# clawrim/gcn10

Measured on AMD Instinct MI355X. Metric: CN Gpixels/sec, higher is better.
Workload: dtype u8

## Files before the change

### gcn10_amd/csrc/gcn10_deflate_fused.hip

```cpp
#include <hip/hip_runtime.h>

#include <cstdint>
#include <cstring>

#include "gcn10_deflate_internal.hpp"
#include "gcn10_gpu.h"
#include "gcn10_gpu_internal.hpp"

using gcn10::as_stream;
using gcn10::fail;
using gcn10::u32x4;
using gcn10::use_device;
using namespace gcn10_deflate;

namespace {

constexpr int kGroup = 6;

struct FusedJob {
    const uint8_t *esa;
    const uint8_t *hx;
    const int32_t *cj;
    const uint8_t *class_of;
    uint16_t *tok;
// ... 1297 lines not shown
            const uint32_t at = (uint32_t)kMaxStream - 4u;
            o[at] = (uint8_t)(adler >> 24);
            o[at + 1] = (uint8_t)(adler >> 16);
            o[at + 2] = (uint8_t)(adler >> 8);
            o[at + 3] = (uint8_t)adler;
        }
        const uint8_t *val = class_val + job.sel[j] * 256;
        const uint32_t xc = (uint32_t)(t & 63) * 4u;
        for (int i = 0; i < kTile / 4; i++) {
            const int r = i * 4 + (t >> 6);
            const uint32_t c4 = class_pixels4(job, tx * kTile + xc, ty * kTile + (uint32_t)r, sh.class_of);
            uint8_t *dst = o + 2 + (r >> 7) * (5 + 32768) + 5 + (r & 127) * kTile + xc;
            dst[0] = val[c4 & 0xffu];
            dst[1] = val[(c4 >> 8) & 0xffu];
            dst[2] = val[(c4 >> 16) & 0xffu];
            dst[3] = val[c4 >> 24];
        }
    }
}

}

extern "C" {

int gcn10_gpu_deflate_fused_available(gcn10_gpu_ctx *ctx)
{
    return ctx && ctx->n_tables > 0 && ctx->n_classes > 0 ? 1 : 0;
}

int gcn10_gpu_deflate_fused_strip(gcn10_gpu_ctx *ctx, const uint8_t *esa, int W, int rows, const int32_t *cj,
                                  unsigned cond_mask, unsigned table_mask, uint8_t *arena_dev, size_t arena_cap,
                                  uint32_t *table_dev, unsigned long long *cursor_dev, gcn10_stream_t stream)
{
    int rc = use_device(ctx);
    if (rc)
        return rc;
    if (ctx->n_tables == 0)
        return fail(GCN10_E_STATE, "gcn10_gpu_deflate_fused_strip: call gcn10_gpu_set_tables first");
    if (ctx->n_classes == 0)
        return fail(GCN10_E_STATE, "gcn10_gpu_deflate_fused_strip: the lookup tables define more than 256 pixel "
                                   "classes; use gcn10_gpu_cn_strip + gcn10_gpu_deflate_strip");
    if (!ctx->d_hx || ctx->hx_W == 0 || (uint32_t)W != ctx->hx_W)
        return fail(GCN10_E_STATE, "gcn10_gpu_deflate_fused_strip: call gcn10_gpu_prepare_tile for W=%d first", W);
    if (W <= 0 || rows < 0 || cond_mask == 0 || (cond_mask & ~3u) || table_mask == 0 ||
        (table_mask >> ctx->n_tables))
        return fail(GCN10_E_INVAL, "gcn10_gpu_deflate_fused_strip: bad shape or masks");
    if (rows == 0)
        return GCN10_OK;
    if (!esa || !cj || !arena_dev || !table_dev || !cursor_dev)
        return fail(GCN10_E_INVAL, "gcn10_gpu_deflate_fused_strip: null pointer");
    if ((reinterpret_cast<uintptr_t>(arena_dev) & 15u) != 0)
        return fail(GCN10_E_INVAL, "gcn10_gpu_deflate_fused_strip: arena must be 16-byte aligned");

    FusedJob job;
    memset(&job, 0, sizeof job);
    job.esa = esa;
    job.hx = ctx->d_hx;
    job.cj = cj;
    job.class_of = ctx->d_class_of;
    job.hx_stride = ctx->hx_stride;
    job.hx_rows = ctx->hx_rows;
    job.seg_align = (uint32_t)ctx->arena_segment_align;
    for (int r = 0; r < GCN10_N_RASTERS; r++)
        if ((cond_mask >> (r / 9)) & 1u && (table_mask >> (r % 9)) & 1u)
            job.sel[job.n_sel++] = (uint8_t)r;
    job.t.arena = arena_dev;
    job.t.table = table_dev;
    job.t.cursor = cursor_dev;
    job.t.W = (uint32_t)W;
    job.t.rows = (uint32_t)rows;
    job.t.across = ((uint32_t)W + kTile - 1) / kTile;
    job.t.down = ((uint32_t)rows + kTile - 1) / kTile;
    if (arena_cap >= 0xfffffffeull)
        return fail(GCN10_E_INVAL, "tile encoder: an arena of %zu bytes does not fit 32-bit stream offsets "
                                   "(use fewer rows per strip)", arena_cap);
    job.t.arena_cap = arena_cap;
    const uint32_t positions = job.t.across * job.t.down;
    if ((uint64_t)positions * (uint64_t)(kMaxStream + kSlotAlign) >= 0xffffffffull)
        return fail(GCN10_E_INVAL, "tile encoder: %u tile positions in one strip (use fewer rows per strip)", positions);
    const uint64_t nblocks = (uint64_t)positions * job.n_sel;
    job.t.n_tiles = (uint32_t)nblocks;

    const size_t stats_bytes = ((size_t)nblocks * ((size_t)kHistWords * 4 + (size_t)kBookBytes) + 255) & ~(size_t)255;
    const size_t tok_bytes = (size_t)positions * kTokStride * sizeof(uint16_t);
    const size_t ntok_bytes = ((size_t)positions * sizeof(uint32_t) + 15) & ~(size_t)15;
    const size_t need = stats_bytes + tok_bytes + ntok_bytes + (size_t)nblocks * 8 + (size_t)job.n_sel * ((positions + 63u) / 64u) * 4;
    rc = gcn10::grow_workspace(&ctx->deflate_ws, &ctx->deflate_ws_cap, need);
    if (rc)
        return rc;
    job.t.hist = reinterpret_cast<uint32_t *>(ctx->deflate_ws);
    job.t.books = reinterpret_cast<uint8_t *>(ctx->deflate_ws) + (size_t)nblocks * kHistWords * 4;
    job.tok = reinterpret_cast<uint16_t *>(reinterpret_cast<uint8_t *>(ctx->deflate_ws) + stats_bytes);
    job.n_tok = reinterpret_cast<uint32_t *>(reinterpret_cast<uint8_t *>(ctx->deflate_ws) + stats_bytes + tok_bytes);
    job.t.sizes = table_dev;
    if (ctx->fused_emit != 0) {
        job.t.sizes = reinterpret_cast<uint32_t *>(reinterpret_cast<uint8_t *>(ctx->deflate_ws) + stats_bytes + tok_bytes + ntok_bytes);
        job.t.chunk_tot = job.t.sizes + (size_t)nblocks * 2;
        job.t.n_chunks = (positions + 63u) / 64u;
    }

    static_assert(sizeof(SharedFA) <= 80 * 1024, "two fused statistics workgroups per CU");
    static_assert(sizeof(SharedFA2) <= 80 * 1024, "two segment-parallel statistics workgroups (32 waves) per CU");
    static_assert(sizeof(SharedFC) <= 20 * 1024, "eight fused emit workgroups per CU");
    static_assert(sizeof(SharedFC2) <= 16 * 1024, "ten wave-independent emit workgroups per CU by LDS");
    if (!ctx->fused_ready) {
        HIP_TRY(hipFuncSetAttribute(reinterpret_cast<const void *>(fused_stats_kernel),
// ... 28 lines not shown
```

### gcn10_amd/csrc/gcn10_gpu.hip

```cpp

#include <hip/hip_runtime.h>
#include <unistd.h>
#include <hip/hip_ext.h>

#include <cstdarg>
#include <cstdint>
#include <cstdio>
#include <cstdlib>
#include <cstring>
#include <new>

#include "gcn10_gpu.h"
#include "gcn10_gpu_internal.hpp"

using gcn10::as_stream;
using gcn10::fail;
using gcn10::u32x4;
using gcn10::use_device;

namespace {

constexpr int kThreads = 256;
constexpr int kPxPerLane = 16;
constexpr int kChunk = kThreads * kPxPerLane;
// ... 358 lines not shown
            }
        }
    }
}

__global__ __launch_bounds__(kThreads) void stream_copy_kernel(const u32x4 *in, u32x4 *out, uint32_t nvec,
                                                               uint32_t ntrips)
{
    uint32_t step, end;
    for (uint32_t trip = first_chunk(ntrips, step, end, true); trip < end; trip += step) {
        u32x4 v[2];
        uint32_t idx[2];
#pragma unroll
        for (int u = 0; u < 2; u++) {
            idx[u] = (trip * 2u + u) * (uint32_t)kThreads + threadIdx.x;
            v[u] = __builtin_nontemporal_load(in + (idx[u] < nvec ? idx[u] : 0u));
        }
#pragma unroll
        for (int u = 0; u < 2; u++)
            if (idx[u] < nvec)
                __builtin_nontemporal_store(v[u], out + idx[u]);
    }
}

__global__ __launch_bounds__(kThreads) void cn_strip_bytes(const StripParams p,
                                                           uint32_t cond_mask)
{
    __shared__ __attribute__((aligned(16))) uint8_t lut[kLut16Bytes];
    for (int i = threadIdx.x; i < kLut16Bytes; i += kThreads)
        lut[i] = p.lut[i];
    __syncthreads();

    const uint32_t stride = gridDim.x * blockDim.x;
    for (uint32_t i = blockIdx.x * blockDim.x + threadIdx.x; i < p.npix; i += stride) {
        const uint32_t y = i / p.W;
        const uint32_t x = i - y * p.W;
        const uint32_t lc = p.esa[i];
        const uint32_t cd = p.hx[(size_t)soil_row(p, y) * p.hx_stride + x];
        for (int c = 0; c < 2; c++) {
            if (!(cond_mask & (1u << c)))
                continue;
            const uint32_t s = (cd >> (4 * c)) & 0xfu;
            const uint8_t *row = lut + s * (uint32_t)kPlane16 + lc * 16u;
            for (int k = 0; k < 9; k++)
                if (p.table_mask & (1u << k))
                    p.out[c * 9 + k][i] = row[k];
        }
    }
}

constexpr uint32_t kExpandRows = 4;

template <bool VEC>
__global__ __launch_bounds__(kThreads) void expand_x_codes(const uint8_t *coarse,
                                                           uint32_t hsx, uint32_t hsy,
                                                           const int32_t *ci, uint32_t W,
                                                           uint8_t *hx, uint32_t hx_stride,
                                                           uint32_t *hx4, uint32_t *complex, uint32_t gen)
{
    const uint32_t x = (blockIdx.x * blockDim.x + threadIdx.x) * 16u;
    const uint32_t r0 = blockIdx.y * kExpandRows;
    if (x >= hx_stride || r0 >= hsy)
        return;
    const uint8_t pad = (uint8_t)(kInvalidPlane | (kInvalidPlane << 4));
    uint32_t cx[16];
    if (VEC && x + 16u <= W) {
        const u32x4 *civ = reinterpret_cast<const u32x4 *>(ci + x);
#pragma unroll
        for (int j = 0; j < 4; j++) {
            const u32x4 c4 = civ[j];
#pragma unroll
            for (int q = 0; q < 4; q++)
                cx[4 * j + q] = c4[q] < hsx ? c4[q] : hsx - 1u;
        }
    }
    else {
#pragma unroll
        for (int q = 0; q < 16; q++) {
            const uint32_t xx = x + q;
            const uint32_t c = xx < W ? (uint32_t)ci[xx] : 0u;
            cx[q] = xx < W ? (c < hsx ? c : hsx - 1u) : 0xffffffffu;
        }
    }
    const uint32_t c_lo = cx[0], c_hi = cx[15];
    const uint32_t r1 = r0 + kExpandRows < hsy ? r0 + kExpandRows : hsy;
    uint32_t split = 0;
    bool compact = true, in_set = true;
#pragma unroll
    for (int q = 0; q < 16; q++) {
        const bool lo = cx[q] == c_lo;
        in_set = in_set && (lo || cx[q] == c_hi);
        compact = compact && (lo ? split == (uint32_t)q : cx[q] == c_hi);
        split += lo && split == (uint32_t)q ? 1u : 0u;
    }
    const bool two = c_lo != 0xffffffffu && c_hi != 0xffffffffu && in_set;
    if (hx4 && x < W && !compact && *reinterpret_cast<volatile uint32_t *>(complex) != gen)
        *reinterpret_cast<volatile uint32_t *>(complex) = gen;
    for (uint32_t r = r0; r < r1; r++) {
        const uint8_t *row = coarse + (size_t)r * hsx;
        u32x4 o;
        if (two) {
            const uint32_t code_lo = soil_code(row[c_lo]), code_hi = soil_code(row[c_hi]);
#pragma unroll
            for (int j = 0; j < 4; j++) {
                uint32_t w = 0;
#pragma unroll
                for (int q = 0; q < 4; q++)
                    w |= (cx[4 * j + q] == c_lo ? code_lo : code_hi) << (8 * q);
                o[j] = w;
            }
        }
        else {
#pragma unroll
            for (int j = 0; j < 4; j++) {
                uint32_t w = 0;
#pragma unroll
                for (int q = 0; q < 4; q++) {
                    const uint32_t c = cx[4 * j + q];
                    const uint8_t code = c == 0xffffffffu ? pad : soil_code(row[c]);
                    w |= (uint32_t)code << (8 * q);
                }
                o[j] = w;
            }
        }
        __builtin_nontemporal_store(o, reinterpret_cast<u32x4 *>(hx + (size_t)r * hx_stride + x));
        if (hx4)
            __builtin_nontemporal_store(compact ? (o[0] & 0xffu) | ((o[3] >> 24) << 8) | (split << 16) : 0x00ff0000u,
                                        hx4 + (size_t)r * (hx_stride / 16u) + x / 16u);
    }
}

__global__ __launch_bounds__(kThreads) void resample_rows(const uint8_t *coarse,
                                                          uint32_t hsx,
                                                          const int32_t *ci,
                                                          const int32_t *cj, uint32_t W,
                                                          uint32_t rows, uint8_t *out)
{
    const size_t npix = (size_t)W * rows;
    const size_t stride = (size_t)gridDim.x * blockDim.x;
    for (size_t i = (size_t)blockIdx.x * blockDim.x + threadIdx.x; i < npix; i += stride) {
        const uint32_t y = (uint32_t)(i / W);
        const uint32_t x = (uint32_t)(i - (size_t)y * W);
        out[i] = coarse[(size_t)(uint32_t)cj[y] * hsx + (uint32_t)ci[x]];
    }
}

__device__ __forceinline__ uint8_t remap_soil(uint8_t h, bool drained)
{
    if (h >= 11 && h <= 14)
        return drained ? (uint8_t)4 : (uint8_t)(h - 10);
    return h;
}

__global__ __launch_bounds__(kThreads) void modify_hysogs_kernel(uint8_t *h, size_t npix,
                                                                 int drained,
                                                                 size_t head, size_t nvec)
{
    const size_t stride = (size_t)gridDim.x * blockDim.x;
    const size_t tid = (size_t)blockIdx.x * blockDim.x + threadIdx.x;
    u32x4 *body = reinterpret_cast<u32x4 *>(h + head);
    for (size_t v = tid; v < nvec; v += stride) {
        u32x4 in = body[v];
        u32x4 o;
#pragma unroll
        for (int j = 0; j < 4; j++) {
            uint32_t w = 0;
#pragma unroll
            for (int q = 0; q < 4; q++)
                w |= (uint32_t)remap_soil((uint8_t)(in[j] >> (8 * q)), drained != 0) << (8 * q);
            o[j] = w;
        }
        body[v] = o;
    }
    const size_t tail0 = head + nvec * 16;
    const size_t nscalar = head + (npix - tail0);
    for (size_t s = tid; s < nscalar; s += stride) {
        const size_t i = s < head ? s : tail0 + (s - head);
        h[i] = remap_soil(h[i], drained != 0);
    }
}

template <bool VEC>
// ... 106 lines not shown
    case 4:
        if (KIND == kLut1)
            return nt ? pick_by_mask<kLut1, 4, true>(cond_mask, all, pf) : pick_by_mask<kLut1, 4, false>(cond_mask, all, pf);
        return nullptr;
    default: return nullptr;
    }
}

strip_kernel_t pick_strip_kernel(bool single, unsigned cond_mask, bool all, int ilp, bool nt, bool pf)
{
    return single ? pick_by_ilp<kLut1>(cond_mask, all, ilp, nt, pf)
                  : pick_by_ilp<kLut16>(cond_mask, all, ilp, nt, pf);
}

}

namespace gcn10 {

thread_local char g_err[512] = "";

int fail(int code, const char *fmt, ...)
{
    va_list ap;
    va_start(ap, fmt);
    vsnprintf(g_err, sizeof g_err, fmt, ap);
    va_end(ap);
    return code;
}

int use_device(gcn10_gpu_ctx *ctx)
{
    if (!ctx)
        return fail(GCN10_E_INVAL, "null context");
    HIP_TRY(hipSetDevice(ctx->device));
    return GCN10_OK;
}

hipStream_t as_stream(gcn10_gpu_ctx *ctx, gcn10_stream_t s)
{
    return s ? reinterpret_cast<hipStream_t>(s) : ctx->main_stream;
}

int grow_workspace(void **ws, size_t *cap, size_t need)
{
    if (need <= *cap)
        return GCN10_OK;
    HIP_TRY(hipDeviceSynchronize());
    if (*ws)
        HIP_TRY(hipFree(*ws));
    *ws = nullptr;
    *cap = 0;
    HIP_TRY(hipMalloc(ws, need));
    *cap = need;
    return GCN10_OK;
}

}

namespace {

uint32_t stream_grid(const gcn10_gpu_ctx *ctx, uint64_t nchunks, int blocks_per_cu = 0)
{
    uint64_t cap = (uint64_t)ctx->n_cus * (blocks_per_cu > 0 ? blocks_per_cu : ctx->grid_blocks_per_cu);
    cap -= cap % 8u;
    if (cap < 8)
        cap = 8;
    uint64_t g = nchunks < cap ? nchunks : cap;
    return (uint32_t)(g ? g : 1);
}

}

extern "C" {

int gcn10_gpu_abi_version(void)
{
    return GCN10_GPU_ABI_VERSION;
}

const char *gcn10_gpu_last_error(void)
{
    return gcn10::g_err;
}

int gcn10_gpu_device_count(void)
{
    int n = 0;
    if (hipGetDeviceCount(&n) != hipSuccess)
        return 0;
    return n;
}

int gcn10_gpu_init(int device, gcn10_gpu_ctx **out)
{
    if (!out)
        return fail(GCN10_E_INVAL, "gcn10_gpu_init: null out pointer");
    *out = nullptr;
    int n = 0;
    hipError_t e = hipGetDeviceCount(&n);
    if (e != hipSuccess || n <= 0)
        return fail(GCN10_E_NODEVICE, "no HIP device visible (%s); this engine has no CPU fallback",
                    e != hipSuccess ? hipGetErrorString(e) : "device count 0");
    if (device < 0 || device >= n)
        return fail(GCN10_E_INVAL, "device %d out of range (0..%d)", device, n - 1);
    HIP_TRY(hipSetDevice(device));
    hipDeviceProp_t prop;
    HIP_TRY(hipGetDeviceProperties(&prop, device));
    if (strncmp(prop.gcnArchName, "gfx950", 6) != 0)
        return fail(GCN10_E_NODEVICE, "device %d is %s; this library carries gfx950 code only",
                    device, prop.gcnArchName);

    gcn10_gpu_ctx *ctx = new (std::nothrow) gcn10_gpu_ctx();
    if (!ctx)
        return fail(GCN10_E_NOMEM, "context allocation failed");
    ctx->device = device;
    ctx->n_cus = prop.multiProcessorCount;
    hipError_t e2 = hipStreamCreateWithFlags(&ctx->main_stream, hipStreamNonBlocking);
    if (e2 == hipSuccess)
        e2 = hipMalloc(reinterpret_cast<void **>(&ctx->d_lut16), kLut16Bytes);
    if (e2 == hipSuccess)
        e2 = hipMalloc(reinterpret_cast<void **>(&ctx->d_lut1), GCN10_N_TABLES * kLut1Bytes);
    if (e2 != hipSuccess) {
        int rc = fail(GCN10_E_HIP, "context setup: %s", hipGetErrorString(e2));
        gcn10_gpu_destroy(ctx);
        return rc;
    }
    *out = ctx;
    return GCN10_OK;
}

void gcn10_gpu_destroy(gcn10_gpu_ctx *ctx)
{
    if (!ctx)
        return;
    (void)hipSetDevice(ctx->device);
    if (ctx->main_stream) {
        (void)hipStreamSynchronize(ctx->main_stream);
        (void)hipStreamDestroy(ctx->main_stream);
    }
    if (ctx->d_lut16)
        (void)hipFree(ctx->d_lut16);
    if (ctx->d_lut1)
        (void)hipFree(ctx->d_lut1);
    if (ctx->d_hx_alloc)
        (void)hipFree(ctx->d_hx_alloc);
    if (ctx->deflate_ws)
        (void)hipFree(ctx->deflate_ws);
    if (ctx->inflate_ws)
        (void)hipFree(ctx->inflate_ws);
    if (ctx->lzw_ws)
        (void)hipFree(ctx->lzw_ws);
    if (ctx->d_class_of)
        (void)hipFree(ctx->d_class_of);
    delete ctx;
}

int gcn10_gpu_device_info(gcn10_gpu_ctx *ctx, char *name, size_t cap, size_t *hbm_bytes)
{
    int rc = use_device(ctx);
    if (rc)
        return rc;
    hipDeviceProp_t prop;
    HIP_TRY(hipGetDeviceProperties(&prop, ctx->device));
    if (name && cap)
        snprintf(name, cap, "%s (%s)", prop.name[0] ? prop.name : "AMD GPU", prop.gcnArchName);
    if (hbm_bytes)
        *hbm_bytes = prop.totalGlobalMem;
    return prop.multiProcessorCount;
}

int gcn10_gpu_pci_bus_id(int device, char *buf, size_t cap)
{
    if (!buf || cap < 13)
        return fail(GCN10_E_INVAL, "gcn10_gpu_pci_bus_id: buffer too small");
    HIP_TRY(hipDeviceGetPCIBusId(buf, (int)cap, device));
    return GCN10_OK;
}


int gcn10_gpu_malloc(gcn10_gpu_ctx *ctx, size_t bytes, void **dptr)
{
    int rc = use_device(ctx);
    if (rc)
        return rc;
    if (!dptr)
        return fail(GCN10_E_INVAL, "gcn10_gpu_malloc: null out pointer");
    *dptr = nullptr;
    HIP_TRY(hipMalloc(dptr, bytes ? bytes : 1));
    return GCN10_OK;
}

int gcn10_gpu_free(gcn10_gpu_ctx *ctx, void *dptr)
{
    int rc = use_device(ctx);
    if (rc)
        return rc;
    if (dptr)
        HIP_TRY(hipFree(dptr));
// ... 301 lines not shown
    return GCN10_OK;
}

int gcn10_gpu_calculate_cn(gcn10_gpu_ctx *ctx, const uint8_t *esa, const uint8_t *hsg,
                           size_t npix, int table_index, uint8_t *out, gcn10_stream_t stream)
{
    int rc = use_device(ctx);
    if (rc)
        return rc;
    if (ctx->n_tables == 0)
        return fail(GCN10_E_STATE, "gcn10_gpu_calculate_cn: call gcn10_gpu_set_tables first");
    if (table_index < 0 || table_index >= ctx->n_tables)
        return fail(GCN10_E_INVAL, "gcn10_gpu_calculate_cn: table %d not loaded (have %d)",
                    table_index, ctx->n_tables);
    if (npix == 0)
        return GCN10_OK;
    if (!esa || !hsg || !out)
        return fail(GCN10_E_INVAL, "gcn10_gpu_calculate_cn: null pointer");
    const uint8_t *img = ctx->d_lut1 + (size_t)table_index * kLut1Bytes;
    const bool vec = aligned16(esa) && aligned16(hsg) && aligned16(out);
    const uint64_t work = vec ? (npix / 16 + 2 * kThreads - 1) / (2 * kThreads) + 1
                              : (npix + kThreads - 1) / kThreads;
    const uint32_t grid = stream_grid(ctx, work);
    if (vec)
        hipLaunchKernelGGL(calculate_cn_kernel<true>, dim3(grid), dim3(kThreads), 0,
                           as_stream(ctx, stream), esa, hsg, npix, img, out);
    else
        hipLaunchKernelGGL(calculate_cn_kernel<false>, dim3(grid), dim3(kThreads), 0,
                           as_stream(ctx, stream), esa, hsg, npix, img, out);
    HIP_TRY(hipGetLastError());
    return GCN10_OK;
}


int gcn10_gpu_prepare_tile(gcn10_gpu_ctx *ctx, const uint8_t *coarse, int hsx, int hsy,
                           const int32_t *ci, int W, gcn10_stream_t stream)
{
    int rc = use_device(ctx);
    if (rc)
        return rc;
    if (hsx <= 0 || hsy <= 0 || W <= 0)
        return fail(GCN10_E_INVAL, "gcn10_gpu_prepare_tile: bad shape W=%d soil=%dx%d", W, hsx, hsy);
    if (!coarse || !ci)
        return fail(GCN10_E_INVAL, "gcn10_gpu_prepare_tile: null pointer");
    const uint32_t stride = (((uint32_t)W + 15u) & ~15u) + 16u;
    const size_t need = (size_t)stride * (size_t)hsy;
    if (need > ctx->hx_capacity) {
        HIP_TRY(hipDeviceSynchronize());
        if (ctx->d_hx_alloc)
            HIP_TRY(hipFree(ctx->d_hx_alloc));
        ctx->d_hx_alloc = ctx->d_hx = nullptr;
        ctx->d_hx4 = ctx->d_hx4_complex = nullptr;
        ctx->hx4_ready = false;
        ctx->hx_capacity = 0;
        const size_t need16 = (need + 15) & ~(size_t)15;
        HIP_TRY(hipMalloc(reinterpret_cast<void **>(&ctx->d_hx_alloc), 16 + need16 + need16 / 4 + 16));
        ctx->d_hx = ctx->d_hx_alloc + 16;
        ctx->d_hx4 = reinterpret_cast<uint32_t *>(ctx->d_hx + need16);
        ctx->d_hx4_complex = reinterpret_cast<uint32_t *>(ctx->d_hx + need16 + need16 / 4);
        HIP_TRY(hipMemsetAsync(ctx->d_hx4_complex, 0, 4, as_stream(ctx, stream)));
        ctx->hx4_gen = 0;
        ctx->hx_capacity = need;
    }
    uint32_t *hx4 = ctx->compact_soil ? ctx->d_hx4 : nullptr;
    ctx->hx4_ready = hx4 != nullptr;
    if (hx4 && ++ctx->hx4_gen == 0u)
        ctx->hx4_gen = 1u;
    ctx->hx_stride = stride;
    ctx->hx_W = (uint32_t)W;
    ctx->hx_rows = (uint32_t)hsy;
    dim3 grid((stride / 16 + kThreads - 1) / kThreads, ((uint32_t)hsy + kExpandRows - 1) / kExpandRows);
    if (aligned16(ci))
        hipLaunchKernelGGL(expand_x_codes<true>, grid, dim3(kThreads), 0, as_stream(ctx, stream),
                           coarse, (uint32_t)hsx, (uint32_t)hsy, ci, (uint32_t)W, ctx->d_hx, stride, hx4,
                           ctx->d_hx4_complex, ctx->hx4_gen);
    else
        hipLaunchKernelGGL(expand_x_codes<false>, grid, dim3(kThreads), 0, as_stream(ctx, stream),
                           coarse, (uint32_t)hsx, (uint32_t)hsy, ci, (uint32_t)W, ctx->d_hx, stride, hx4,
                           ctx->d_hx4_complex, ctx->hx4_gen);
    HIP_TRY(hipGetLastError());
    return GCN10_OK;
}

int gcn10_gpu_cn_strip(gcn10_gpu_ctx *ctx, const uint8_t *esa, int W, int rows,
                       const int32_t *cj, unsigned cond_mask, unsigned table_mask,
                       uint8_t *const out[GCN10_N_RASTERS], gcn10_stream_t stream)
{
    int rc = use_device(ctx);
    if (rc)
        return rc;
    if (ctx->n_tables == 0)
        return fail(GCN10_E_STATE, "gcn10_gpu_cn_strip: call gcn10_gpu_set_tables first");
    if (!ctx->d_hx || ctx->hx_W == 0)
        return fail(GCN10_E_STATE, "gcn10_gpu_cn_strip: call gcn10_gpu_prepare_tile first");
    if (W <= 0 || rows < 0 || (uint32_t)W != ctx->hx_W)
        return fail(GCN10_E_INVAL, "gcn10_gpu_cn_strip: W=%d rows=%d does not match prepared tile W=%u",
                    W, rows, ctx->hx_W);
    if ((uint64_t)W * (uint64_t)rows > 0x7fffffffull)
        return fail(GCN10_E_INVAL, "gcn10_gpu_cn_strip: strip of %d x %d exceeds 2^31-1 pixels", W, rows);
    if (cond_mask == 0 || (cond_mask & ~3u))
        return fail(GCN10_E_INVAL, "gcn10_gpu_cn_strip: cond_mask 0x%x", cond_mask);
    if (table_mask == 0 || (table_mask >> ctx->n_tables))
        return fail(GCN10_E_INVAL, "gcn10_gpu_cn_strip: table_mask 0x%x with %d tables loaded",
                    table_mask, ctx->n_tables);
    if (rows == 0)
        return GCN10_OK;
    if (!esa || !cj || !out)
        return fail(GCN10_E_INVAL, "gcn10_gpu_cn_strip: null pointer");

    StripParams p;
    memset(&p, 0, sizeof p);
    bool all_aligned = aligned16(esa);
    for (int c = 0; c < 2; c++) {
        for (int k = 0; k < 9; k++) {
            const int r = c * 9 + k;
            if ((cond_mask & (1u << c)) && (table_mask & (1u << k))) {
                if (!out[r])
                    return fail(GCN10_E_INVAL, "gcn10_gpu_cn_strip: out[%d] is null but selected", r);
                p.out[r] = out[r];
                all_aligned = all_aligned && aligned16(out[r]);
            }
        }
    }
    p.esa = esa;
    p.hx = ctx->d_hx;
    p.cj = cj;
    p.W = (uint32_t)W;
    p.rows = (uint32_t)rows;
    p.npix = (uint32_t)((uint64_t)W * (uint64_t)rows);
    p.hx_stride = ctx->hx_stride;
    p.hx_rows = ctx->hx_rows;
    p.nchunks = (p.npix + kChunk - 1) / kChunk;
    p.table_mask = table_mask;
    hipStream_t s = as_stream(ctx, stream);

    p.xcd_slabs = (uint32_t)ctx->xcd_slabs;
    p.nvec16 = p.npix & ~15u;
    if (ctx->hx4_ready && ctx->compact_soil && (p.W & 15u) == 0u) {
        p.hx4 = ctx->d_hx4;
        p.hx4_complex = ctx->d_hx4_complex;
        p.hx4_stride = ctx->hx_stride / 16u;
        p.hx4_gen = ctx->hx4_gen;
    }
    if (p.npix < 16u || p.W < kMinVectorW)
        all_aligned = false;
    if (!all_aligned) {
        p.lut = ctx->d_lut16;
        const uint32_t g = stream_grid(ctx, ((uint64_t)p.npix + kThreads - 1) / kThreads);
        if (ctx->time_start && ctx->time_stop) {
            void *args[] = { &p, &cond_mask };
            HIP_TRY(hipExtLaunchKernel(reinterpret_cast<const void *>(cn_strip_bytes), dim3(g), dim3(kThreads), args, 0,
                                       s, ctx->time_start, ctx->time_stop, 0));
            ctx->time_start = ctx->time_stop = nullptr;
        }
        else {
            hipLaunchKernelGGL(cn_strip_bytes, dim3(g), dim3(kThreads), 0, s, p, cond_mask);
        }
        ctx->last_kernel = "cn_strip_bytes";
    }
    else {
        const bool single = popcount(table_mask) == 1;
        const bool all = table_mask == 0x1ffu;
        const int n_streams = popcount(cond_mask) * popcount(table_mask);
        const bool tuned = single && ctx->single.set;
        const int ilp = tuned ? ctx->single.ilp
                              : single ? ctx->ilp1 : (ctx->ilp16 > 0 ? ctx->ilp16 : (n_streams > 9 ? 1 : 2));
        const bool nt = ctx->nontemporal != 0;
        if (single) {
            p.single_k = (uint32_t)__builtin_ctz(table_mask);
            p.lut = ctx->d_lut1 + (size_t)p.single_k * kLut1Bytes;
        }
        else {
            p.lut = ctx->d_lut16;
        }
        const bool pf = (tuned ? ctx->single.prefetch : ctx->prefetch) != 0 && ilp <= 2;
        p.nchunks = (p.nchunks + (uint32_t)ilp - 1) / (uint32_t)ilp;
        const uint32_t grid = stream_grid(ctx, p.nchunks, tuned ? ctx->single.grid_blocks_per_cu : 0);
        if (tuned)
            p.xcd_slabs = (uint32_t)ctx->single.xcd_slabs;
        strip_kernel_t fn = pick_strip_kernel(single, cond_mask, all, ilp, nt, pf);
        if (!fn)
            return fail(GCN10_E_INVAL, "gcn10_gpu_cn_strip: no kernel for ilp=%d", ilp);
        if (ctx->time_start && ctx->time_stop) {
            void *args[] = { &p };
            HIP_TRY(hipExtLaunchKernel(reinterpret_cast<const void *>(fn), dim3(grid), dim3(kThreads), args, 0,
                                       s, ctx->time_start, ctx->time_stop, 0));
            ctx->time_start = ctx->time_stop = nullptr;
        }
        else {
            hipLaunchKernelGGL(fn, dim3(grid), dim3(kThreads), 0, s, p);
        }
        snprintf(ctx->kernel_name, sizeof ctx->kernel_name, "cn_strip_kernel<%d, %u, %s, %d, %s, %s>",
                 single ? 1 : 0, cond_mask, (all || single) ? "true" : "false", ilp, nt ? "true" : "false",
                 pf ? "true" : "false");
        ctx->last_kernel = ctx->kernel_name;
    }
    HIP_TRY(hipGetLastError());
    return GCN10_OK;
// ... 218 lines not shown
```

### gcn10_amd/csrc/gcn10_gpu_internal.hpp

```cpp
#ifndef GCN10_GPU_INTERNAL_HPP
#define GCN10_GPU_INTERNAL_HPP

#include <hip/hip_runtime.h>

#include <cstdint>

#include "gcn10_gpu.h"

namespace gcn10 {

int fail(int code, const char *fmt, ...) __attribute__((format(printf, 2, 3)));

#define HIP_TRY(expr)                                                                   \
    do {                                                                                \
        hipError_t e_ = (expr);                                                         \
        if (e_ != hipSuccess)                                                           \
            return gcn10::fail(e_ == hipErrorOutOfMemory ? GCN10_E_NOMEM : GCN10_E_HIP, \
                               "%s: %s", #expr, hipGetErrorString(e_));                 \
    } while (0)

int use_device(gcn10_gpu_ctx *ctx);
hipStream_t as_stream(gcn10_gpu_ctx *ctx, gcn10_stream_t s);
int grow_workspace(void **ws, size_t *cap, size_t need);

typedef uint32_t u32x4 __attribute__((ext_vector_type(4)));

__device__ __forceinline__ bool inflate_window_ok(uint32_t out_len, uint32_t chunk_w, uint32_t src_x, uint32_t src_y,
                                                  uint32_t copy_w, uint32_t copy_h, uint32_t slot_bytes)
{
    if (copy_w == 0 || copy_h == 0)
        return true;
    if (chunk_w == 0 || out_len > slot_bytes || src_x > chunk_w || copy_w > chunk_w - src_x)
        return false;
    const unsigned long long last = (unsigned long long)(src_y + copy_h - 1u) * chunk_w + src_x + copy_w;
    return (unsigned long long)src_y + copy_h <= 0xffffffffull && last <= out_len;
}

void launch_lzw_decode(const uint8_t *comp_dev, const gcn10_inflate_tile *tiles_dev, uint32_t n_tiles,
                       uint8_t *scratch, uint32_t slot_bytes, uint32_t *status_dev, hipStream_t stream);

constexpr int kClassCodes = 36;

constexpr int kLut16Plane = 256 * 16 + 16;
constexpr int kLut16Bytes = 6 * kLut16Plane;

}

struct gcn10_gpu_ctx {
    int device = -1;
    int n_cus = 0;
    hipStream_t main_stream = nullptr;
    uint8_t *d_lut16 = nullptr;
    uint8_t *d_lut1 = nullptr;
    int n_tables = 0;
    uint8_t *d_hx = nullptr;
    uint8_t *d_hx_alloc = nullptr;
    uint32_t *d_hx4 = nullptr;
    uint32_t *d_hx4_complex = nullptr;
    uint32_t hx4_gen = 0;
    bool hx4_ready = false;
    int compact_soil = 1;
    size_t hx_capacity = 0;
    uint32_t hx_stride = 0;
    uint32_t hx_W = 0;
    uint32_t hx_rows = 0;
    const char *last_kernel = "";
    char kernel_name[96] = "";
    int grid_blocks_per_cu = 16;
    int ilp16 = 0;
    int ilp1 = 2;
    int nontemporal = 1;
    int xcd_slabs = 1;
    int prefetch = 1;
    struct SingleShape {
        bool set = false;
        int xcd_slabs = 1, grid_blocks_per_cu = 8, ilp = 2, prefetch = 1;
    } single;
    hipEvent_t time_start = nullptr, time_stop = nullptr;
    uint8_t *d_class_of = nullptr;
    int n_classes = 0;
    int arena_segment_align = 4096;
    int deflate_wave_codes = 1;
    int fused_parse = 1;
    int fused_emit = 1;
    int event_sync_sleep_us = 0;
    bool fused_ready = false;
    bool codes_ready = false;
    bool deflate_ready = false;
    void *deflate_ws = nullptr;
    size_t deflate_ws_cap = 0;
    void *inflate_ws = nullptr;
    size_t inflate_ws_cap = 0;
    void *lzw_ws = nullptr;
    size_t lzw_ws_cap = 0;
};

#endif
```

### gcn10_amd/csrc/gcn10_overview.hip

```cpp
#include <hip/hip_runtime.h>

#include <cstdint>

#include "gcn10_gpu_internal.hpp"

using namespace gcn10;

namespace {

constexpr int kThreads = 256;
constexpr int kPlanes = 6;
constexpr int kPlane16 = 256 * 16 + 16;
constexpr int kLut16Bytes = kPlanes * kPlane16;
constexpr int kMaxLevels = 8;
constexpr int kL1Tile = 128;
constexpr uint32_t kL1Rows = 4;

__device__ __forceinline__ uint8_t avg_of(uint32_t s, uint32_t n)
{
    return n == 0 ? (uint8_t)GCN10_NODATA : (uint8_t)((2u * s + n) / (2u * n));
}

struct NearestParams {
    const uint8_t *src;
// ... 131 lines not shown
        cur = nxt;
        nxt = t;
        Wl = Wk;
        Hl = Hk;
        w = wk;
        h = hk;
        side = sidek;
    }
}

}

extern "C" {

int gcn10_gpu_overview_nearest(gcn10_gpu_ctx *ctx, const uint8_t *src, int W, int H, int level, uint8_t *dst,
                               gcn10_stream_t stream)
{
    int rc = use_device(ctx);
    if (rc)
        return rc;
    if (!src || !dst || W <= 0 || H <= 0 || level < 1 || level > 30)
        return fail(GCN10_E_INVAL, "gcn10_gpu_overview_nearest: bad arguments W=%d H=%d level=%d", W, H, level);
    NearestParams p;
    p.src = src;
    p.dst = dst;
    p.W = (uint32_t)W;
    p.H = (uint32_t)H;
    p.level = (uint32_t)level;
    p.Wk = (uint32_t)(((int64_t)W + (1ll << level) - 1) >> level);
    p.Hk = (uint32_t)(((int64_t)H + (1ll << level) - 1) >> level);
    dim3 grid((p.Wk + kThreads - 1) / kThreads, p.Hk);
    hipLaunchKernelGGL(overview_nearest_kernel, grid, dim3(kThreads), 0, as_stream(ctx, stream), p);
    HIP_TRY(hipGetLastError());
    return GCN10_OK;
}

int gcn10_gpu_overview_average(gcn10_gpu_ctx *ctx, const uint8_t *esa, int W, int H, int y0, int rows,
                               const int32_t *cj, unsigned cond_mask, unsigned table_mask, int n_levels,
                               uint8_t *const *levels, gcn10_stream_t stream)
{
    int rc = use_device(ctx);
    if (rc)
        return rc;
    if (ctx->n_tables == 0)
        return fail(GCN10_E_STATE, "gcn10_gpu_overview_average: call gcn10_gpu_set_tables first");
    if (!ctx->d_hx || (int)ctx->hx_W != W)
        return fail(GCN10_E_STATE, "gcn10_gpu_overview_average: prepare the block's tile (W=%d) first", W);
    if (!esa || !cj || !levels || W <= 0 || H <= 0 || n_levels < 1 || n_levels > kMaxLevels || y0 < 0 ||
        rows <= 0 || y0 % 256 != 0 || y0 + rows > H || (rows % 256 != 0 && y0 + rows != H))
        return fail(GCN10_E_INVAL, "gcn10_gpu_overview_average: bad strip y0=%d rows=%d of %dx%d, %d levels "
                    "(strips start and end on multiples of 256 rows, 1..8 levels)", y0, rows, W, H, n_levels);
    if (cond_mask == 0 || (cond_mask & ~3u) || table_mask == 0 || (table_mask >> ctx->n_tables) != 0)
        return fail(GCN10_E_INVAL, "gcn10_gpu_overview_average: bad masks cond=%#x table=%#x", cond_mask, table_mask);
    AvgParams p = {};
    p.esa = esa;
    p.cj = cj;
    p.lut16 = ctx->d_lut16;
    p.hx = ctx->d_hx;
    p.hx_stride = ctx->hx_stride;
    p.hx_rows = ctx->hx_rows;
    p.W = (uint32_t)W;
    p.H = (uint32_t)H;
    p.cond_mask = cond_mask;
    p.table_mask = table_mask;
    p.n_levels = (uint32_t)n_levels;
    int q = 0;
    for (int r = 0; r < GCN10_N_RASTERS; r++) {
        if (!((cond_mask >> (r / 9)) & 1u) || !((table_mask >> (r % 9)) & 1u))
            continue;
        for (int k = 0; k < n_levels; k++) {
            p.out[r][k] = levels[q * n_levels + k];
            if (!p.out[r][k])
                return fail(GCN10_E_INVAL, "gcn10_gpu_overview_average: level %d of raster %d is NULL", k + 1, r);
        }
        q++;
    }
    const uint32_t W1 = ((uint32_t)W + 1u) >> 1;
    p.y1_begin = (uint32_t)y0 / 2u;
    p.y1_end = ((uint32_t)(y0 + rows) + 1u) / 2u;
    hipStream_t s = as_stream(ctx, stream);
    dim3 grid1((W1 + kThreads - 1) / kThreads, (p.y1_end - p.y1_begin + kL1Rows - 1) / kL1Rows);
    hipLaunchKernelGGL(overview_avg_level1_kernel, grid1, dim3(kThreads), 0, s, p);
    HIP_TRY(hipGetLastError());
    if (n_levels >= 2) {
        const uint32_t ty0 = (uint32_t)y0 / 256u, ty1 = ((uint32_t)(y0 + rows) + 255u) / 256u;
        dim3 grid2((W1 + kL1Tile - 1) / kL1Tile, ty1 - ty0, GCN10_N_RASTERS);
        hipLaunchKernelGGL(overview_avg_deeper_kernel, grid2, dim3(kThreads), 0, s, p, ty0);
        HIP_TRY(hipGetLastError());
    }
    return GCN10_OK;
}

}
```

### gcn10_amd/csrc/gcn10_stats.hip

```cpp
#include <hip/hip_runtime.h>

#include <cstdint>

#include "gcn10_gpu_internal.hpp"

using namespace gcn10;

namespace {

constexpr int kThreads = 256;
constexpr uint32_t kPxPerLane = 16;
constexpr uint32_t kChunk = kThreads * kPxPerLane;
constexpr int kBins = GCN10_PAIR_HIST_BINS;
constexpr int kHistWords = GCN10_PAIR_HIST_SIZE;
constexpr uint32_t kRowsPerItem = 4;
constexpr int kGridPerCu = 4;

__host__ __device__ inline uint32_t code_bin(uint32_t code)
{
    const uint32_t d = code & 15u, u = code >> 4;
    const uint32_t b = d == u ? d : 5u + u;
    return b < (uint32_t)kBins ? b : (uint32_t)kBins - 1u;
}

// ... 93 lines not shown
        if (x0 + kPxPerLane <= p.W) {
            typedef u32x4 u32x4_u __attribute__((aligned(1)));
            u32x4 e[kRowsPerItem], s[kRowsPerItem];
#pragma unroll
            for (uint32_t j = 0; j < kRowsPerItem; j++) {
                e[j] = *reinterpret_cast<const u32x4_u *>(erow[j]);
                s[j] = *reinterpret_cast<const u32x4 *>(srow[j]);
            }
#pragma unroll
            for (uint32_t j = 0; j < kRowsPerItem; j++)
                if (j < ny)
                    count16(h, e[j], s[j]);
        }
        else {
            for (uint32_t j = 0; j < ny; j++)
                count_tail(h, erow[j], srow[j], p.W - x0);
        }
    }
    __syncthreads();
    for (uint32_t i = threadIdx.x; i < (uint32_t)kHistWords; i += kThreads)
        if (h[i])
            atomicAdd(&p.hist[i], (unsigned long long)h[i]);
}

}

extern "C" {

int gcn10_gpu_pair_histogram_codes(uint8_t codes[GCN10_PAIR_HIST_BINS])
{
    if (!codes)
        return fail(GCN10_E_INVAL, "gcn10_gpu_pair_histogram_codes: null pointer");
    for (int b = 0; b < kBins; b++)
        codes[b] = 0x55;
    for (uint32_t d = 0; d <= 5; d++)
        codes[code_bin(d | d << 4)] = (uint8_t)(d | d << 4);
    for (uint32_t u = 1; u <= 3; u++)
        codes[code_bin(4u | u << 4)] = (uint8_t)(4u | u << 4);
    return GCN10_PAIR_HIST_BINS;
}

int gcn10_gpu_pair_histogram(gcn10_gpu_ctx *ctx, const uint8_t *esa, int W, int rows, const int32_t *cj,
                             unsigned long long *hist_dev, gcn10_stream_t stream)
{
    int rc = use_device(ctx);
    if (rc)
        return rc;
    if (!ctx->d_hx || (int)ctx->hx_W != W)
        return fail(GCN10_E_STATE, "gcn10_gpu_pair_histogram: prepare the block's tile (W=%d) first", W);
    if (!esa || !cj || !hist_dev || W <= 0 || rows < 0)
        return fail(GCN10_E_INVAL, "gcn10_gpu_pair_histogram: bad arguments W=%d rows=%d", W, rows);
    if (rows == 0)
        return GCN10_OK;
    HistParams p = {};
    p.esa = esa;
    p.hx = ctx->d_hx;
    p.cj = cj;
    p.hist = hist_dev;
    p.W = (uint32_t)W;
    p.rows = (uint32_t)rows;
    p.hx_stride = ctx->hx_stride;
    p.hx_rows = ctx->hx_rows;
    p.per_row = ((uint32_t)W + kChunk - 1u) / kChunk;
    const uint64_t items = (uint64_t)((p.rows + kRowsPerItem - 1u) / kRowsPerItem) * p.per_row;
    const uint64_t cap = (uint64_t)(ctx->n_cus > 0 ? ctx->n_cus : 256) * kGridPerCu;
    const uint32_t grid = (uint32_t)(items < cap ? items : cap);
    hipLaunchKernelGGL(pair_histogram_kernel, dim3(grid), dim3(kThreads), 0, as_stream(ctx, stream), p);
    HIP_TRY(hipGetLastError());
    return GCN10_OK;
}

}
```

### gcn10_amd/csrc/gcn10_verify.hip

```cpp
#include <hip/hip_runtime.h>

#include <cstdint>
#include <cstring>

#include "gcn10_gpu_internal.hpp"

using namespace gcn10;

namespace {

constexpr int kThreads = 256;
constexpr uint32_t kPxPerLane = 16;
constexpr int kGridPerCu = 4;

struct VerifyParams {
    const uint8_t *esa;
    const uint8_t *hx;
    const int32_t *cj;
    const uint8_t *lut;
    const uint8_t *want[GCN10_N_RASTERS];
    const uint8_t *got[GCN10_N_RASTERS];
    gcn10_verify_count *counts;
    uint64_t want_stride, got_stride;
    uint32_t W, rows, y0;
// ... 287 lines not shown
    p.groups_per_row = p.W / kPxPerLane;
    p.n_groups = p.rows * p.groups_per_row;
    return GCN10_OK;
}

}

extern "C" {

int gcn10_gpu_verify_strip(gcn10_gpu_ctx *ctx, const uint8_t *esa, int W, int rows, const int32_t *cj,
                           unsigned cond_mask, unsigned table_mask, const uint8_t *const got[GCN10_N_RASTERS],
                           size_t got_stride, int y0, gcn10_verify_count *counts_dev, gcn10_stream_t stream)
{
    int rc = use_device(ctx);
    if (rc)
        return rc;
    if (!ctx->d_lut16 || ctx->n_tables == 0)
        return fail(GCN10_E_STATE, "gcn10_gpu_verify_strip: call gcn10_gpu_set_tables first");
    if (!ctx->d_hx || (int)ctx->hx_W != W)
        return fail(GCN10_E_STATE, "gcn10_gpu_verify_strip: prepare the block's tile (W=%d) first", W);
    if (cond_mask == 0 || (cond_mask & ~3u))
        return fail(GCN10_E_INVAL, "gcn10_gpu_verify_strip: cond_mask 0x%x", cond_mask);
    if (table_mask == 0 || (table_mask >> ctx->n_tables))
        return fail(GCN10_E_INVAL, "gcn10_gpu_verify_strip: table_mask 0x%x with %d tables loaded", table_mask,
                    ctx->n_tables);
    VerifyParams p;
    memset(&p, 0, sizeof p);
    rc = fill_shape(p, "gcn10_gpu_verify_strip", W, rows, y0, got_stride);
    if (rc)
        return rc;
    if (rows == 0)
        return GCN10_OK;
    if (!esa || !cj || !got || !counts_dev)
        return fail(GCN10_E_INVAL, "gcn10_gpu_verify_strip: null pointer");
    for (int c = 0; c < GCN10_N_CONDS; c++) {
        for (int k = 0; k < GCN10_N_TABLES; k++) {
            const int r = c * GCN10_N_TABLES + k;
            if (!(cond_mask & (1u << c)) || !(table_mask & (1u << k)))
                continue;
            if (!got[r])
                return fail(GCN10_E_INVAL, "gcn10_gpu_verify_strip: got[%d] is null but selected", r);
            p.got[r] = got[r];
            p.sel |= 1u << r;
        }
    }
    p.esa = esa;
    p.hx = ctx->d_hx;
    p.cj = cj;
    p.lut = ctx->d_lut16;
    p.counts = counts_dev;
    p.hx_stride = ctx->hx_stride;
    p.hx_rows = ctx->hx_rows;
    hipStream_t s = as_stream(ctx, stream);
    if (p.sel == (1u << GCN10_N_RASTERS) - 1u)
        hipLaunchKernelGGL(verify_strip_kernel<true>, dim3(grid_for(ctx, p)), dim3(kThreads), 0, s, p);
    else
        hipLaunchKernelGGL(verify_strip_kernel<false>, dim3(grid_for(ctx, p)), dim3(kThreads), 0, s, p);
    HIP_TRY(hipGetLastError());
    hipLaunchKernelGGL(verify_first_kernel<true>, dim3(1), dim3(64), 0, s, p);
    HIP_TRY(hipGetLastError());
    return GCN10_OK;
}

int gcn10_gpu_verify_buffers(gcn10_gpu_ctx *ctx, const uint8_t *const want[GCN10_N_RASTERS], size_t want_stride,
                             const uint8_t *const got[GCN10_N_RASTERS], size_t got_stride, int W, int rows, int y0,
                             unsigned raster_mask, gcn10_verify_count *counts_dev, gcn10_stream_t stream)
{
    int rc = use_device(ctx);
    if (rc)
        return rc;
    if (raster_mask == 0 || (raster_mask >> GCN10_N_RASTERS))
        return fail(GCN10_E_INVAL, "gcn10_gpu_verify_buffers: raster_mask 0x%x", raster_mask);
    VerifyParams p;
    memset(&p, 0, sizeof p);
    rc = fill_shape(p, "gcn10_gpu_verify_buffers", W, rows, y0, got_stride);
    if (rc)
        return rc;
    if (want_stride < (size_t)W)
        return fail(GCN10_E_INVAL, "gcn10_gpu_verify_buffers: want_stride %zu < W=%d", want_stride, W);
    if (rows == 0)
        return GCN10_OK;
    if (!want || !got || !counts_dev)
        return fail(GCN10_E_INVAL, "gcn10_gpu_verify_buffers: null pointer");
    for (int r = 0; r < GCN10_N_RASTERS; r++) {
        if (!(raster_mask & (1u << r)))
            continue;
        if (!want[r] || !got[r])
            return fail(GCN10_E_INVAL, "gcn10_gpu_verify_buffers: raster %d is selected but has a null pointer", r);
        p.want[r] = want[r];
        p.got[r] = got[r];
    }
    p.sel = raster_mask;
    p.want_stride = want_stride;
    p.counts = counts_dev;
    hipStream_t s = as_stream(ctx, stream);
    hipLaunchKernelGGL(verify_buffers_kernel, dim3(grid_for(ctx, p)), dim3(kThreads), 0, s, p);
    HIP_TRY(hipGetLastError());
    hipLaunchKernelGGL(verify_first_kernel<false>, dim3(1), dim3(64), 0, s, p);
    HIP_TRY(hipGetLastError());
    return GCN10_OK;
}

}
```

Measured before the change: 2925.

## Build only compact soil words at tile prep, materialize byte codes lazily

Tile preparation now launches a per-row-block scan kernel that classifies each 16-pixel group once in shared memory and writes only the compact hx4 words, skipping the full byte-code expansion unless the column mapping is complex. A lazy ensure_soil_bytes step rebuilds the byte plane from the words on demand, tracked with a validity flag and event, before any consumer that needs bytes (deflate, verify, overview, histogram, unaligned CN). This removes the byte-plane write from the common CN path but adds an extra kernel and event wait for byte consumers and shared-memory limits on width.

```diff
diff --git a/gcn10_amd/csrc/gcn10_deflate_fused.hip b/gcn10_amd/csrc/gcn10_deflate_fused.hip
--- a/gcn10_amd/csrc/gcn10_deflate_fused.hip
+++ b/gcn10_amd/csrc/gcn10_deflate_fused.hip
@@ -1373,6 +1373,10 @@
     if ((reinterpret_cast<uintptr_t>(arena_dev) & 15u) != 0)
         return fail(GCN10_E_INVAL, "gcn10_gpu_deflate_fused_strip: arena must be 16-byte aligned");
 
+    rc = gcn10::ensure_soil_bytes(ctx, as_stream(ctx, stream));
+    if (rc)
+        return rc;
+
     FusedJob job;
     memset(&job, 0, sizeof job);
     job.esa = esa;
diff --git a/gcn10_amd/csrc/gcn10_gpu.hip b/gcn10_amd/csrc/gcn10_gpu.hip
--- a/gcn10_amd/csrc/gcn10_gpu.hip
+++ b/gcn10_amd/csrc/gcn10_gpu.hip
@@ -434,14 +434,11 @@
 constexpr uint32_t kExpandRows = 4;
 
 template <bool VEC>
-__global__ __launch_bounds__(kThreads) void expand_x_codes(const uint8_t *coarse,
-                                                           uint32_t hsx, uint32_t hsy,
-                                                           const int32_t *ci, uint32_t W,
-                                                           uint8_t *hx, uint32_t hx_stride,
-                                                           uint32_t *hx4, uint32_t *complex, uint32_t gen)
-{
-    const uint32_t x = (blockIdx.x * blockDim.x + threadIdx.x) * 16u;
-    const uint32_t r0 = blockIdx.y * kExpandRows;
+__device__ __forceinline__ void expand_x_group(const uint8_t *coarse, uint32_t hsx, uint32_t hsy,
+                                               const int32_t *ci, uint32_t W, uint8_t *hx, uint32_t hx_stride,
+                                               uint32_t *hx4, uint32_t *complex, uint32_t gen,
+                                               uint32_t x, uint32_t r0)
+{
     if (x >= hx_stride || r0 >= hsy)
         return;
     const uint8_t pad = (uint8_t)(kInvalidPlane | (kInvalidPlane << 4));
@@ -510,6 +507,104 @@
             __builtin_nontemporal_store(compact ? (o[0] & 0xffu) | ((o[3] >> 24) << 8) | (split << 16) : 0x00ff0000u,
                                         hx4 + (size_t)r * (hx_stride / 16u) + x / 16u);
     }
+}
+
+template <bool VEC>
+__global__ __launch_bounds__(kThreads) void expand_x_codes(const uint8_t *coarse,
+                                                           uint32_t hsx, uint32_t hsy,
+                                                           const int32_t *ci, uint32_t W,
+                                                           uint8_t *hx, uint32_t hx_stride,
+                                                           uint32_t *hx4, uint32_t *complex, uint32_t gen)
+{
+    expand_x_group<VEC>(coarse, hsx, hsy, ci, W, hx, hx_stride, hx4, complex, gen,
+                        (blockIdx.x * blockDim.x + threadIdx.x) * 16u, blockIdx.y * kExpandRows);
+}
+
+constexpr uint32_t kScanRows = kExpandRows;
+constexpr uint32_t kScanGroups = 4096;
+
+template <bool VEC>
+__global__ __launch_bounds__(kThreads) void soil_words_scan(const uint8_t *coarse, uint32_t hsx, uint32_t hsy,
+                                                            const int32_t *ci, uint32_t W, uint8_t *hx,
+                                                            uint32_t hx_stride, uint32_t *hx4, uint32_t *complex,
+                                                            uint32_t gen)
+{
+    __shared__ uint32_t s_lo[kScanGroups], s_hi[kScanGroups];
+    __shared__ uint8_t s_split[kScanGroups];
+    const uint32_t ngroups = W / 16u;
+    bool bad = false;
+#pragma unroll 3
+    for (uint32_t g = threadIdx.x; g < ngroups; g += kThreads) {
+        uint32_t cx[16];
+        if (VEC) {
+            const u32x4 *civ = reinterpret_cast<const u32x4 *>(ci + g * 16u);
+#pragma unroll
+            for (int j = 0; j < 4; j++) {
+                const u32x4 c4 = civ[j];
+#pragma unroll
+                for (int q = 0; q < 4; q++)
+                    cx[4 * j + q] = c4[q] < hsx ? c4[q] : hsx - 1u;
+            }
+        }
+        else {
+#pragma unroll
+            for (int q = 0; q < 16; q++) {
+                const uint32_t c = (uint32_t)ci[g * 16u + q];
+                cx[q] = c < hsx ? c : hsx - 1u;
+            }
+        }
+        const uint32_t c_lo = cx[0], c_hi = cx[15];
+        uint32_t split = 0;
+        bool compact = true;
+#pragma unroll
+        for (int q = 0; q < 16; q++) {
+            const bool lo = cx[q] == c_lo;
+            compact = compact && (lo ? split == (uint32_t)q : cx[q] == c_hi);
+            split += lo && split == (uint32_t)q ? 1u : 0u;
+        }
+        s_lo[g] = c_lo;
+        s_hi[g] = c_hi;
+        s_split[g] = (uint8_t)(compact ? split : 0xffu);
+        bad = bad || !compact;
+    }
+    const bool complex_tile = __syncthreads_or(bad) != 0;
+
+    const uint32_t r0 = blockIdx.x * kScanRows;
+    const uint32_t hx4_stride = hx_stride / 16u;
+    const uint32_t pad = (uint32_t)(kInvalidPlane | (kInvalidPlane << 4));
+#pragma unroll 3
+    for (uint32_t g = threadIdx.x; g <= ngroups; g += kThreads) {
+        const bool behind = g == ngroups;
+        const uint32_t split = behind ? 16u : s_split[g];
+        const uint32_t c_lo = behind ? 0u : s_lo[g], c_hi = behind ? 0u : s_hi[g];
+        uint32_t w[kScanRows];
+#pragma unroll
+        for (uint32_t k = 0; k < kScanRows; k++) {
+            const uint8_t *row = coarse + (size_t)(r0 + k < hsy ? r0 + k : hsy - 1u) * hsx;
+            w[k] = (uint32_t)soil_code(row[c_lo]) | ((uint32_t)soil_code(row[c_hi]) << 8) | (split << 16);
+        }
+#pragma unroll
+        for (uint32_t k = 0; k < kScanRows; k++)
+            if (r0 + k < hsy)
+                __builtin_nontemporal_store(behind ? pad | (pad << 8) | (16u << 16) : split == 0xffu ? 0x00ff0000u : w[k],
+                                            hx4 + (size_t)(r0 + k) * hx4_stride + g);
+    }
+    if (!complex_tile)
+        return;
+    if (blockIdx.x == 0 && threadIdx.x == 0)
+        *reinterpret_cast<volatile uint32_t *>(complex) = gen;
+    for (uint32_t x = threadIdx.x * 16u; x < hx_stride; x += kThreads * 16u)
+        expand_x_group<VEC>(coarse, hsx, hsy, ci, W, hx, hx_stride, nullptr, nullptr, gen, x, r0);
+}
+
+__global__ __launch_bounds__(kThreads) void soil_bytes_from_words(const uint32_t *hx4, uint32_t n, u32x4 *hx,
+                                                                  const uint32_t *complex, uint32_t gen)
+{
+    if (*reinterpret_cast<const volatile uint32_t *>(complex) == gen)
+        return;
+    const uint32_t stride = gridDim.x * blockDim.x;
+    for (uint32_t i = blockIdx.x * blockDim.x + threadIdx.x; i < n; i += stride)
+        hx[i] = expand_soil_word(hx4[i]);
 }
 
 __global__ __launch_bounds__(kThreads) void resample_rows(const uint8_t *coarse,
@@ -722,6 +817,30 @@
     *cap = 0;
     HIP_TRY(hipMalloc(ws, need));
     *cap = need;
+    return GCN10_OK;
+}
+
+int ensure_soil_bytes(gcn10_gpu_ctx *ctx, hipStream_t stream)
+{
+    if (ctx->hx_bytes_valid) {
+        if (ctx->hx_bytes_event_live)
+            HIP_TRY(hipStreamWaitEvent(stream, ctx->hx_bytes_event, 0));
+        return GCN10_OK;
+    }
+    if (!ctx->hx4_ready || !ctx->d_hx || !ctx->d_hx4)
+        return fail(GCN10_E_STATE, "soil code bytes: no prepared tile to rebuild them from");
+    if (!ctx->hx_bytes_event)
+        HIP_TRY(hipEventCreateWithFlags(&ctx->hx_bytes_event, hipEventDisableTiming));
+    const uint64_t n = (uint64_t)(ctx->hx_stride / 16u) * ctx->hx_rows;
+    if (n > 0x7fffffffull)
+        return fail(GCN10_E_INVAL, "soil code bytes: tile of %u x %u groups is too large", ctx->hx_stride / 16u, ctx->hx_rows);
+    const uint64_t cap = (uint64_t)(ctx->n_cus > 0 ? ctx->n_cus : 256) * 8u;
+    const uint64_t wgs = (n + kThreads - 1) / kThreads;
+    hipLaunchKernelGGL(soil_bytes_from_words, dim3((uint32_t)(wgs < cap ? wgs : cap)), dim3(kThreads), 0, stream,
+                       ctx->d_hx4, (uint32_t)n, reinterpret_cast<u32x4 *>(ctx->d_hx), ctx->d_hx4_complex, ctx->hx4_gen);
+    HIP_TRY(hipGetLastError());
+    HIP_TRY(hipEventRecord(ctx->hx_bytes_event, stream));
+    ctx->hx_bytes_valid = ctx->hx_bytes_event_live = true;
     return GCN10_OK;
 }
 
@@ -814,6 +933,8 @@
         (void)hipFree(ctx->d_lut1);
     if (ctx->d_hx_alloc)
         (void)hipFree(ctx->d_hx_alloc);
+    if (ctx->hx_bytes_event)
+        (void)hipEventDestroy(ctx->hx_bytes_event);
     if (ctx->deflate_ws)
         (void)hipFree(ctx->deflate_ws);
     if (ctx->inflate_ws)
@@ -1221,6 +1342,7 @@
         ctx->d_hx_alloc = ctx->d_hx = nullptr;
         ctx->d_hx4 = ctx->d_hx4_complex = nullptr;
         ctx->hx4_ready = false;
+        ctx->hx_bytes_valid = ctx->hx_bytes_event_live = false;
         ctx->hx_capacity = 0;
         const size_t need16 = (need + 15) & ~(size_t)15;
         HIP_TRY(hipMalloc(reinterpret_cast<void **>(&ctx->d_hx_alloc), 16 + need16 + need16 / 4 + 16));
@@ -1238,7 +1360,24 @@
     ctx->hx_stride = stride;
     ctx->hx_W = (uint32_t)W;
     ctx->hx_rows = (uint32_t)hsy;
-    dim3 grid((stride / 16 + kThreads - 1) / kThreads, ((uint32_t)hsy + kExpandRows - 1) / kExpandRows);
+    ctx->hx_bytes_event_live = false;
+    const uint32_t gx = (stride / 16 + kThreads - 1) / kThreads;
+    if (hx4 && ((uint32_t)W & 15u) == 0u && (uint32_t)W / 16u <= kScanGroups) {
+        ctx->hx_bytes_valid = false;
+        const dim3 gs(((uint32_t)hsy + kScanRows - 1) / kScanRows);
+        if (aligned16(ci))
+            hipLaunchKernelGGL(soil_words_scan<true>, gs, dim3(kThreads), 0, as_stream(ctx, stream), coarse,
+                               (uint32_t)hsx, (uint32_t)hsy, ci, (uint32_t)W, ctx->d_hx, stride, hx4,
+                               ctx->d_hx4_complex, ctx->hx4_gen);
+        else
+            hipLaunchKernelGGL(soil_words_scan<false>, gs, dim3(kThreads), 0, as_stream(ctx, stream), coarse,
+                               (uint32_t)hsx, (uint32_t)hsy, ci, (uint32_t)W, ctx->d_hx, stride, hx4,
+                               ctx->d_hx4_complex, ctx->hx4_gen);
+        HIP_TRY(hipGetLastError());
+        return GCN10_OK;
+    }
+    ctx->hx_bytes_valid = true;
+    dim3 grid(gx, ((uint32_t)hsy + kExpandRows - 1) / kExpandRows);
     if (aligned16(ci))
         hipLaunchKernelGGL(expand_x_codes<true>, grid, dim3(kThreads), 0, as_stream(ctx, stream),
                            coarse, (uint32_t)hsx, (uint32_t)hsy, ci, (uint32_t)W, ctx->d_hx, stride, hx4,
@@ -1313,6 +1452,11 @@
     }
     if (p.npix < 16u || p.W < kMinVectorW)
         all_aligned = false;
+    if (!all_aligned || !p.hx4) {
+        rc = gcn10::ensure_soil_bytes(ctx, s);
+        if (rc)
+            return rc;
+    }
     if (!all_aligned) {
         p.lut = ctx->d_lut16;
         const uint32_t g = stream_grid(ctx, ((uint64_t)p.npix + kThreads - 1) / kThreads);
diff --git a/gcn10_amd/csrc/gcn10_gpu_internal.hpp b/gcn10_amd/csrc/gcn10_gpu_internal.hpp
--- a/gcn10_amd/csrc/gcn10_gpu_internal.hpp
+++ b/gcn10_amd/csrc/gcn10_gpu_internal.hpp
@@ -24,6 +24,8 @@
 int grow_workspace(void **ws, size_t *cap, size_t need);
 
 typedef uint32_t u32x4 __attribute__((ext_vector_type(4)));
+
+int ensure_soil_bytes(gcn10_gpu_ctx *ctx, hipStream_t stream);
 
 __device__ __forceinline__ bool inflate_window_ok(uint32_t out_len, uint32_t chunk_w, uint32_t src_x, uint32_t src_y,
                                                   uint32_t copy_w, uint32_t copy_h, uint32_t slot_bytes)
@@ -60,6 +62,9 @@
     uint32_t hx4_gen = 0;
     bool hx4_ready = false;
     int compact_soil = 1;
+    bool hx_bytes_valid = false;
+    bool hx_bytes_event_live = false;
+    hipEvent_t hx_bytes_event = nullptr;
     size_t hx_capacity = 0;
     uint32_t hx_stride = 0;
     uint32_t hx_W = 0;
diff --git a/gcn10_amd/csrc/gcn10_overview.hip b/gcn10_amd/csrc/gcn10_overview.hip
--- a/gcn10_amd/csrc/gcn10_overview.hip
+++ b/gcn10_amd/csrc/gcn10_overview.hip
@@ -207,6 +207,9 @@
                     "(strips start and end on multiples of 256 rows, 1..8 levels)", y0, rows, W, H, n_levels);
     if (cond_mask == 0 || (cond_mask & ~3u) || table_mask == 0 || (table_mask >> ctx->n_tables) != 0)
         return fail(GCN10_E_INVAL, "gcn10_gpu_overview_average: bad masks cond=%#x table=%#x", cond_mask, table_mask);
+    rc = gcn10::ensure_soil_bytes(ctx, as_stream(ctx, stream));
+    if (rc)
+        return rc;
     AvgParams p = {};
     p.esa = esa;
     p.cj = cj;
diff --git a/gcn10_amd/csrc/gcn10_stats.hip b/gcn10_amd/csrc/gcn10_stats.hip
--- a/gcn10_amd/csrc/gcn10_stats.hip
+++ b/gcn10_amd/csrc/gcn10_stats.hip
@@ -169,6 +169,9 @@
         return fail(GCN10_E_INVAL, "gcn10_gpu_pair_histogram: bad arguments W=%d rows=%d", W, rows);
     if (rows == 0)
         return GCN10_OK;
+    rc = gcn10::ensure_soil_bytes(ctx, as_stream(ctx, stream));
+    if (rc)
+        return rc;
     HistParams p = {};
     p.esa = esa;
     p.hx = ctx->d_hx;
diff --git a/gcn10_amd/csrc/gcn10_verify.hip b/gcn10_amd/csrc/gcn10_verify.hip
--- a/gcn10_amd/csrc/gcn10_verify.hip
+++ b/gcn10_amd/csrc/gcn10_verify.hip
@@ -363,6 +363,9 @@
     p.hx_stride = ctx->hx_stride;
     p.hx_rows = ctx->hx_rows;
     hipStream_t s = as_stream(ctx, stream);
+    rc = gcn10::ensure_soil_bytes(ctx, s);
+    if (rc)
+        return rc;
     if (p.sel == (1u << GCN10_N_RASTERS) - 1u)
         hipLaunchKernelGGL(verify_strip_kernel<true>, dim3(grid_for(ctx, p)), dim3(kThreads), 0, s, p);
     else
```

Result: slower. 2880 (-1.6%).
